# AhmedKishki/AMP-SPARC-SpatialModulation

Measured on AMD Instinct MI355X. Metric: detected symbol-vectors/sec, VAMP Nt=256 Nr=512 16-QAM; SER match vs ref, higher is better.
Workload: dtype bf16x3; 1 GPU; cfg4: VAMP Nt=256 Nr=512 Na=8 16QAM batch=4096 iterations<=20 EbN0=8.0 dB, one channel per batch; global_batch=4096, parallelism=epoch-shard x1 (independent epochs, one all-reduce of the error counters)

## Files before the change

### amp-sparc-spatialmodulation_amd/csrc/amp_persist.h

```cpp
#pragma once

#include <cfloat>

#include "amp_common.h"

namespace amp {

constexpr int PRING = 4;

typedef float f32x4 __attribute__((ext_vector_type(4)));
typedef unsigned u32x4 __attribute__((ext_vector_type(4)));

__device__ __forceinline__ f32x4 mfma16x16x4(float a, float b, f32x4 c) {
    return __builtin_amdgcn_mfma_f32_16x16x4f32(a, b, c, 0, 0, 0);
}

template <int NT, int G>
__device__ __forceinline__ void gemm16(const float* sA, int lda, const float* __restrict__ wq, int ct0,
                                       f32x4 (&acc)[NT]) {
    constexpr int R = G < PRING ? G : PRING;
    const int lane = threadIdx.x & 63;
#pragma unroll
    for (int t = 0; t < NT; ++t) acc[t] = f32x4{0.f, 0.f, 0.f, 0.f};
    const int ct0u = __builtin_amdgcn_readfirstlane(ct0);
    const __amdgpu_buffer_rsrc_t wr = __builtin_amdgcn_make_buffer_rsrc(
        const_cast<float*>(wq) + (size_t)ct0u * G * 256, (short)0, 0x7ffffff0, 0x00020000);
    const int vo = lane * 16;
    auto wload = [&](int t, int g) {
        const f32x4 v = __builtin_amdgcn_raw_buffer_load_b128(wr, vo, (t * G + g) * 1024, 0);
        return make_float4(v.x, v.y, v.z, v.w);
    };
    float4 ring[R][NT];
#pragma unroll
    for (int d = 0; d < R; ++d)
#pragma unroll
        for (int t = 0; t < NT; ++t) ring[d][t] = wload(t, d);
    const float* a_s = sA + (lane & 15) * lda + 4 * (lane >> 4);
    float4 acur = *reinterpret_cast<const float4*>(a_s);
#pragma unroll
    for (int g = 0; g < G; ++g) {
        const int d = g % R;
        const float4 anext = *reinterpret_cast<const float4*>(a_s + 16 * (g + 1 < G ? g + 1 : g));
#pragma unroll
        for (int t = 0; t < NT; ++t) acc[t] = mfma16x16x4(acur.x, ring[d][t].x, acc[t]);
#pragma unroll
        for (int t = 0; t < NT; ++t) acc[t] = mfma16x16x4(acur.y, ring[d][t].y, acc[t]);
#pragma unroll
        for (int t = 0; t < NT; ++t) acc[t] = mfma16x16x4(acur.z, ring[d][t].z, acc[t]);
#pragma unroll
        for (int t = 0; t < NT; ++t) acc[t] = mfma16x16x4(acur.w, ring[d][t].w, acc[t]);
        if (g + R < G) {
#pragma unroll
            for (int t = 0; t < NT; ++t) ring[d][t] = wload(t, g + R);
        }
        acur = anext;
        __builtin_amdgcn_sched_barrier(0);
    }
}

__host__ __device__ inline int pl_ldx(int K) { return K; }
__device__ __forceinline__ int pl_mask(int ldx) {
    const int n = ldx >> 3;
    const int b = n & -n;
    return (b < 16 ? b : 16) - 1;
}
__device__ __forceinline__ int pl_col(int row, int j, int m) { return j ^ ((row & m) << 3); }
__device__ __forceinline__ int pl_opaque(int x) {
#ifndef AMP_PL_HOIST
    asm volatile("" : "+v"(x));
#endif
    return x;
}

typedef const __attribute__((address_space(4))) char* KargPtr;
template <class A, class B>
constexpr int karg_second_offset() {
    return (int)((sizeof(A) + alignof(B) - 1) / alignof(B) * alignof(B));
}
template <class T>
__device__ __forceinline__ const T* karg_at(unsigned long long base, int off) {
    return (const T*)(const __attribute__((address_space(4))) T*)(KargPtr)(base + (unsigned long long)off);
}
__device__ __forceinline__ unsigned long long karg_launder(unsigned long long v) {
    asm volatile("" : "+s"(v));
    return v;
}
__device__ __forceinline__ unsigned long long karg_base() {
    return (unsigned long long)(KargPtr)__builtin_amdgcn_kernarg_segment_ptr();
}

typedef __bf16 bf16x8 __attribute__((ext_vector_type(8)));

typedef __bf16 bf16x2_t __attribute__((ext_vector_type(2)));
typedef float f32x2_t __attribute__((ext_vector_type(2)));

__device__ __forceinline__ void split3x2(float x, float y, unsigned& p0, unsigned& p1, unsigned& p2) {
    const f32x2_t v = {x, y};
    const bf16x2_t b0 = __builtin_convertvector(v, bf16x2_t);
    f32x2_t r1 = v - __builtin_convertvector(b0, f32x2_t);
    r1.x = __builtin_isfinite(x) ? r1.x : 0.0f;
    r1.y = __builtin_isfinite(y) ? r1.y : 0.0f;
    const bf16x2_t b1 = __builtin_convertvector(r1, bf16x2_t);
    const f32x2_t r2 = r1 - __builtin_convertvector(b1, f32x2_t);
    const bf16x2_t b2 = __builtin_convertvector(r2, bf16x2_t);
    p0 = __builtin_bit_cast(unsigned, b0);
    p1 = __builtin_bit_cast(unsigned, b1);
    p2 = __builtin_bit_cast(unsigned, b2);
}

__device__ __forceinline__ void x3_store8(unsigned short* sP, int ldx, int row, int j0, const float (&re)[8],
                                          const float (&im)[8]) {
    u32x4 q[6];
#pragma unroll
    for (int h = 0; h < 4; ++h) {
        unsigned a0, a1, a2, b0, b1, b2;
        split3x2(re[2 * h], re[2 * h + 1], a0, a1, a2);
        split3x2(im[2 * h], im[2 * h + 1], b0, b1, b2);
        q[0][h] = a0; q[1][h] = a1; q[2][h] = a2; q[3][h] = b0; q[4][h] = b1; q[5][h] = b2;
    }
    const int c = pl_col(pl_opaque(row), j0, pl_mask(ldx));
#pragma unroll
    for (int f = 0; f < 6; ++f) *reinterpret_cast<u32x4*>(sP + (f * 16 + row) * ldx + c) = q[f];
}

__device__ __forceinline__ float dpp_swap_pair(float v) {
    return __int_as_float(__builtin_amdgcn_update_dpp(0, __float_as_int(v), 0xB1, 0xF, 0xF, false));
}

__device__ __forceinline__ void x3_store_acc(unsigned short* sP, int ldx, int o, const float (&vr)[4],
                                             const float (&vi)[4]) {
    const int lane = pl_opaque((int)threadIdx.x) & 63;
    const bool odd = (lane & 1) != 0;
    float gr[2], gi[2];
#pragma unroll
    for (int h = 0; h < 2; ++h) {
        gr[h] = dpp_swap_pair(odd ? vr[h] : vr[2 + h]);
        gi[h] = dpp_swap_pair(odd ? vi[h] : vi[2 + h]);
    }
    const int row0 = 4 * (lane >> 4) + (odd ? 2 : 0);
    const int m = pl_mask(ldx);
    const int pl = 16 * ldx;
#pragma unroll
    for (int h = 0; h < 2; ++h) {
        unsigned short* p = sP + (row0 + h) * ldx + pl_col(row0 + h, o & ~1, m);
        const float mr = odd ? vr[2 + h] : vr[h], mi = odd ? vi[2 + h] : vi[h];
        unsigned q[6];
        split3x2(odd ? gr[h] : mr, odd ? mr : gr[h], q[0], q[1], q[2]);
        split3x2(odd ? gi[h] : mi, odd ? mi : gi[h], q[3], q[4], q[5]);
#pragma unroll
        for (int f = 0; f < 6; ++f) *reinterpret_cast<unsigned*>(p + f * pl) = q[f];
    }
}

__device__ __forceinline__ void split3(float x, unsigned& p0, unsigned& p1, unsigned& p2) {
    unsigned q0, q1, q2;
    split3x2(x, 0.0f, q0, q1, q2);
    p0 = q0 & 0xffffu; p1 = q1 & 0xffffu; p2 = q2 & 0xffffu;
}

__device__ __forceinline__ bf16x8 as_bf16x8(u32x4 v) { return __builtin_bit_cast(bf16x8, v); }

template <int NT, int G, int R = 1, bool PIN = false, bool HL = false>
__device__ __forceinline__ void gemm_x3(const unsigned short* sP, int ldx, const void* __restrict__ wq, int ct0,
                                        f32x4 (&cr)[NT], f32x4 (&ci)[NT]) {
    constexpr int RR = G < R ? G : R;
    constexpr int NL = HL ? NT : 1;
    const int lane = threadIdx.x & 63;
    f32x4 lr[NL], li[NL];
#pragma unroll
    for (int t = 0; t < NT; ++t) { cr[t] = f32x4{0.f, 0.f, 0.f, 0.f}; ci[t] = f32x4{0.f, 0.f, 0.f, 0.f}; }
#pragma unroll
    for (int t = 0; t < NL; ++t) { lr[t] = f32x4{0.f, 0.f, 0.f, 0.f}; li[t] = f32x4{0.f, 0.f, 0.f, 0.f}; }
    const int ct0u = __builtin_amdgcn_readfirstlane(ct0);
    const __amdgpu_buffer_rsrc_t wr = __builtin_amdgcn_make_buffer_rsrc(
        (char*)const_cast<void*>(wq) + (size_t)ct0u * G * 6 * 1024, (short)0, 0x7ffffff0, 0x00020000);
    const int vo = lane * 16;
    u32x4 ring[RR][NT][6];
#pragma unroll
    for (int d = 0; d < RR; ++d)
#pragma unroll
        for (int t = 0; t < NT; ++t)
#pragma unroll
            for (int f = 0; f < 6; ++f)
                ring[d][t][f] = __builtin_amdgcn_raw_buffer_load_b128(wr, vo, ((t * G + d) * 6 + f) * 1024, 0);
    const int ln = pl_opaque(lane);
    const int sw = (ln & 15) & pl_mask(ldx);
    const unsigned short* ap = sP + (ln & 15) * ldx + 8 * ((ln >> 4) ^ (sw & 3));
    const int s32 = 32 * (sw >> 2);
    const u32x4 sgn = {0x80008000u, 0x80008000u, 0x80008000u, 0x80008000u};
    u32x4 an[6];
    if constexpr (!PIN) {
#pragma unroll
        for (int f = 0; f < 6; ++f) an[f] = *reinterpret_cast<const u32x4*>(ap + s32 + f * 16 * ldx);
    }
#pragma unroll
    for (int g = 0; g < G; ++g) {
        const int d = g % RR;
        u32x4 a[6], na[3];
        if constexpr (PIN) {
#pragma unroll
            for (int f = 0; f < 6; ++f) a[f] = *reinterpret_cast<const u32x4*>(ap + ((32 * g) ^ s32) + f * 16 * ldx);
        } else {
#pragma unroll
            for (int f = 0; f < 6; ++f) a[f] = an[f];
            if (g + 1 < G) {
#pragma unroll
                for (int f = 0; f < 6; ++f)
                    an[f] = *reinterpret_cast<const u32x4*>(ap + ((32 * (g + 1)) ^ s32) + f * 16 * ldx);
            }
        }
#pragma unroll
        for (int f = 0; f < 3; ++f) na[f] = a[3 + f] ^ sgn;
#pragma unroll
        for (int t = 0; t < NT; ++t) {
            const u32x4* w = ring[d][t];
            f32x4 gr = cr[t], gi = ci[t];
            f32x4 sr = HL ? lr[HL ? t : 0] : gr, si = HL ? li[HL ? t : 0] : gi;
#define AMP_MF(acc, x, y) acc = __builtin_amdgcn_mfma_f32_16x16x32_bf16(as_bf16x8(x), as_bf16x8(y), acc, 0, 0, 0)
            AMP_MF(sr, a[0], w[2]);  AMP_MF(si, a[0], w[5]);
            AMP_MF(sr, a[1], w[1]);  AMP_MF(si, a[1], w[4]);
            AMP_MF(sr, a[2], w[0]);  AMP_MF(si, a[2], w[3]);
            AMP_MF(sr, na[0], w[5]); AMP_MF(si, a[3], w[2]);
            AMP_MF(sr, na[1], w[4]); AMP_MF(si, a[4], w[1]);
            AMP_MF(sr, na[2], w[3]); AMP_MF(si, a[5], w[0]);
            AMP_MF(sr, a[0], w[1]);  AMP_MF(si, a[0], w[4]);
            AMP_MF(sr, a[1], w[0]);  AMP_MF(si, a[1], w[3]);
            AMP_MF(sr, na[0], w[4]); AMP_MF(si, a[3], w[1]);
            AMP_MF(sr, na[1], w[3]); AMP_MF(si, a[4], w[0]);
            if constexpr (HL) {
                lr[HL ? t : 0] = sr; li[HL ? t : 0] = si;
            } else {
                gr = sr; gi = si;
            }
            AMP_MF(gr, a[0], w[0]);  AMP_MF(gi, a[0], w[3]);
            AMP_MF(gr, na[0], w[3]); AMP_MF(gi, a[3], w[0]);
#undef AMP_MF
            cr[t] = gr; ci[t] = gi;
        }
        if constexpr (PIN) __builtin_amdgcn_sched_barrier(0);
        if (g + RR < G) {
#pragma unroll
            for (int t = 0; t < NT; ++t)
#pragma unroll
                for (int f = 0; f < 6; ++f)
                    ring[d][t][f] = __builtin_amdgcn_raw_buffer_load_b128(wr, vo, ((t * G + g + RR) * 6 + f) * 1024, 0);
        }
        __builtin_amdgcn_sched_barrier(0);
    }
    if constexpr (HL) {
#pragma unroll
        for (int t = 0; t < NT; ++t) { cr[t] += lr[HL ? t : 0]; ci[t] += li[HL ? t : 0]; }
    }
}

typedef _Float16 f16x8 __attribute__((ext_vector_type(8)));
typedef _Float16 f16x2_t __attribute__((ext_vector_type(2)));
constexpr int H2_EX = 14;
constexpr int YH2_EX = 10;

__device__ __forceinline__ int h2_row_exp(float m) {
    if (!(m > 0.f) || !__builtin_isfinite(m)) return 0;
    return 14 - __builtin_amdgcn_frexp_expf(m);
}

__device__ __forceinline__ void split2x2(float x, float y, unsigned& p0, unsigned& p1) {
    const f32x2_t v = {x, y};
    const f16x2_t h0 = __builtin_convertvector(v, f16x2_t);
    const f32x2_t b = __builtin_convertvector(h0, f32x2_t);
    f32x2_t r = v - b;
    r.x = __builtin_isfinite(b.x) ? r.x : 0.0f;
    r.y = __builtin_isfinite(b.y) ? r.y : 0.0f;
    const f16x2_t h1 = __builtin_convertvector(r, f16x2_t);
    p0 = __builtin_bit_cast(unsigned, h0);
    p1 = __builtin_bit_cast(unsigned, h1);
}

__device__ __forceinline__ void split2(float x, int e, unsigned& p0, unsigned& p1) {
    unsigned q0, q1;
    split2x2(__builtin_amdgcn_ldexpf(x, e), 0.0f, q0, q1);
    p0 = q0 & 0xffffu; p1 = q1 & 0xffffu;
}

__device__ __forceinline__ void h2_store8(unsigned short* sP, int ldx, int row, int j0, const float (&re)[8],
                                          const float (&im)[8]) {
    u32x4 q[4];
#pragma unroll
    for (int h = 0; h < 4; ++h) {
        unsigned a0, a1, b0, b1;
        split2x2(re[2 * h], re[2 * h + 1], a0, a1);
        split2x2(im[2 * h], im[2 * h + 1], b0, b1);
        q[0][h] = a0; q[1][h] = a1; q[2][h] = b0; q[3][h] = b1;
    }
    const int c = pl_col(pl_opaque(row), j0, pl_mask(ldx));
#pragma unroll
    for (int f = 0; f < 4; ++f) *reinterpret_cast<u32x4*>(sP + (f * 16 + row) * ldx + c) = q[f];
}

__device__ __forceinline__ void h2_store_acc(unsigned short* sP, int ldx, int o, const float (&vr)[4],
                                             const float (&vi)[4]) {
    const int lane = pl_opaque((int)threadIdx.x) & 63;
    const bool odd = (lane & 1) != 0;
    float gr[2], gi[2];
#pragma unroll
    for (int h = 0; h < 2; ++h) {
        gr[h] = dpp_swap_pair(odd ? vr[h] : vr[2 + h]);
        gi[h] = dpp_swap_pair(odd ? vi[h] : vi[2 + h]);
    }
    const int row0 = 4 * (lane >> 4) + (odd ? 2 : 0);
    const int m = pl_mask(ldx);
    const int pl = 16 * ldx;
#pragma unroll
    for (int h = 0; h < 2; ++h) {
        unsigned short* p = sP + (row0 + h) * ldx + pl_col(row0 + h, o & ~1, m);
        const float mr = odd ? vr[2 + h] : vr[h], mi = odd ? vi[2 + h] : vi[h];
        unsigned q[4];
        split2x2(odd ? gr[h] : mr, odd ? mr : gr[h], q[0], q[1]);
        split2x2(odd ? gi[h] : mi, odd ? mi : gi[h], q[2], q[3]);
#pragma unroll
        for (int f = 0; f < 4; ++f) *reinterpret_cast<unsigned*>(p + f * pl) = q[f];
    }
}

__device__ __forceinline__ f16x8 as_f16x8(u32x4 v) { return __builtin_bit_cast(f16x8, v); }

template <int NT, int G, int R = 1>
__device__ __forceinline__ void gemm_h2(const unsigned short* sP, int ldx, const void* __restrict__ wq, int ct0,
                                        f32x4 (&cr)[NT], f32x4 (&ci)[NT]) {
    constexpr int RR = G < R ? G : R;
    const int lane = threadIdx.x & 63;
#pragma unroll
    for (int t = 0; t < NT; ++t) { cr[t] = f32x4{0.f, 0.f, 0.f, 0.f}; ci[t] = f32x4{0.f, 0.f, 0.f, 0.f}; }
    const int ct0u = __builtin_amdgcn_readfirstlane(ct0);
    const __amdgpu_buffer_rsrc_t wr = __builtin_amdgcn_make_buffer_rsrc(
        (char*)const_cast<void*>(wq) + (size_t)ct0u * G * 4 * 1024, (short)0, 0x7ffffff0, 0x00020000);
    const int vo = lane * 16;
    u32x4 ring[RR][NT][4];
#pragma unroll
    for (int d = 0; d < RR; ++d)
#pragma unroll
        for (int t = 0; t < NT; ++t)
#pragma unroll
            for (int f = 0; f < 4; ++f)
                ring[d][t][f] = __builtin_amdgcn_raw_buffer_load_b128(wr, vo, ((t * G + d) * 4 + f) * 1024, 0);
    const int ln = pl_opaque(lane);
    const int sw = (ln & 15) & pl_mask(ldx);
    const unsigned short* ap = sP + (ln & 15) * ldx + 8 * ((ln >> 4) ^ (sw & 3));
    const int s32 = 32 * (sw >> 2);
    const u32x4 sgn = {0x80008000u, 0x80008000u, 0x80008000u, 0x80008000u};
    u32x4 an[4];
#pragma unroll
    for (int f = 0; f < 4; ++f) an[f] = *reinterpret_cast<const u32x4*>(ap + s32 + f * 16 * ldx);
#pragma unroll
    for (int g = 0; g < G; ++g) {
        const int d = g % RR;
        u32x4 a[4], na[2];
#pragma unroll
        for (int f = 0; f < 4; ++f) a[f] = an[f];
        if (g + 1 < G) {
#pragma unroll
            for (int f = 0; f < 4; ++f)
                an[f] = *reinterpret_cast<const u32x4*>(ap + ((32 * (g + 1)) ^ s32) + f * 16 * ldx);
        }
#pragma unroll
        for (int f = 0; f < 2; ++f) na[f] = a[2 + f] ^ sgn;
#pragma unroll
        for (int t = 0; t < NT; ++t) {
            const u32x4* w = ring[d][t];
#define AMP_MH(acc, x, y) acc = __builtin_amdgcn_mfma_f32_16x16x32_f16(as_f16x8(x), as_f16x8(y), acc, 0, 0, 0)
            AMP_MH(cr[t], a[0], w[1]);  AMP_MH(ci[t], a[0], w[3]);
            AMP_MH(cr[t], a[1], w[0]);  AMP_MH(ci[t], a[1], w[2]);
            AMP_MH(cr[t], na[0], w[3]); AMP_MH(ci[t], a[2], w[1]);
            AMP_MH(cr[t], na[1], w[2]); AMP_MH(ci[t], a[3], w[0]);
            AMP_MH(cr[t], a[0], w[0]);  AMP_MH(ci[t], a[0], w[2]);
            AMP_MH(cr[t], na[0], w[2]); AMP_MH(ci[t], a[2], w[0]);
#undef AMP_MH
        }
        if (g + RR < G) {
#pragma unroll
            for (int t = 0; t < NT; ++t)
#pragma unroll
                for (int f = 0; f < 4; ++f)
                    ring[d][t][f] = __builtin_amdgcn_raw_buffer_load_b128(wr, vo, ((t * G + g + RR) * 4 + f) * 1024, 0);
        }
        __builtin_amdgcn_sched_barrier(0);
    }
}

typedef int i32x4 __attribute__((ext_vector_type(4)));
#ifndef AMP_I8_APF
#define AMP_I8_APF 1
#endif
__host__ __device__ __forceinline__ size_t i8_exp_offset(int O, int J) { return (size_t)O * J * 8; }

__host__ __device__ __forceinline__ int i8_ldb(int N) { return N + 16; }
__host__ __device__ __forceinline__ int i8_plane_floats(int N) { return 8 * 16 * i8_ldb(N) / 4; }

__device__ __forceinline__ int i8_row_exp(float m) {
    if (!(m <= FLT_MAX)) return 0x7fffffff;
    if (!(m > 0.f)) return 0;
    return __builtin_amdgcn_frexp_expf(m);
}
__device__ __forceinline__ float i8_absmax(float m, float v) {
    const float a = fabsf(v);
    return fmaxf(m, a <= FLT_MAX ? a : INFINITY);
}
// ... 262 lines not shown
```

### amp-sparc-spatialmodulation_amd/csrc/amp_vamp_persist_kernel.h

```cpp
#pragma once

#include <stdlib.h>

#include <type_traits>

#include "amp_decide_fused.h"
#include "amp_persist.h"
#include "amp_vamp.h"

namespace amp {

constexpr int AMP_TRACE_STRIDE = 10;
#ifndef AMP_OCC2_PK
#define AMP_OCC2_PK 0
#endif
#ifndef AMP_KK4_DU
#define AMP_KK4_DU 4
#endif
#ifndef AMP_X3_W8_PIN
#define AMP_X3_W8_PIN 0
#endif
#ifndef AMP_X3_W8_RING
#define AMP_X3_W8_RING 1
#endif
#ifndef AMP_X3_W8_PKGRID
#define AMP_X3_W8_PKGRID 1
#endif
#ifndef AMP_X3_DU
#define AMP_X3_DU 2
#endif

struct PLayout {
    int lda, ldr;
    int offA, offR, offX, offV0, offV1, offSM, offSA, offScr, total;
};

__host__ __device__ inline int x3_ldx(int N) { return pl_ldx(N); }
__host__ __device__ inline int x3_plane_floats(int N) { return 6 * 16 * x3_ldx(N) / 2; }

__host__ __device__ inline PLayout playout(int N, int k, int L, bool x3 = false) {
    PLayout y;
    y.lda = (2 * N > 2 * k ? 2 * N : 2 * k) + 4;
    y.ldr = 2 * N + (x3 ? 8 : 4);
    int o = 0;
    y.offA = o; o += (x3 && x3_plane_floats(N) > PBM * y.lda) ? x3_plane_floats(N) : PBM * y.lda;
    y.offR = o; o += PBM * y.ldr;
    y.offX = o; o += PBM * y.ldr;
    y.offV0 = o; o += PBM * N;
    y.offV1 = o; o += PBM * N;
    y.offSM = o; o += PBM * L;
    y.offSA = o; o += PBM * L;
    o = (o + 3) & ~3;
    y.offScr = o; o += 1024;
    y.total = o;
    return y;
}

constexpr int KARG_DC_OFF = karg_second_offset<VampK, DecConst>();

template <int NT, int KK, int NWV, int DU, bool X3, int OCC = 1, bool H2 = false, bool I8 = false>
__global__ __launch_bounds__(64 * NWV, OCC * NWV / 4) void vamp_persist(VampK P_arg, DecConst dc_arg) {
    (void)P_arg;
    (void)dc_arg;
    unsigned long long kbase = karg_base();
    const VampK* Pp = karg_at<VampK>(kbase, 0);
    const DecConst* Dp = karg_at<DecConst>(kbase, KARG_DC_OFF);
#define P (*Pp)
#define dc (*Dp)
    static_assert(!X3 || ((NWV == 4 || (NWV == 8 && !H2 && OCC == 1)) && NT % 2 == 0),
                  "X3: four waves (eight for the bf16x3 two-waves-per-SIMD form), whole complex tiles");
    static_assert(!(H2 && I8) && (!I8 || X3), "I8: a split-precision form of its own");
    constexpr int PKDEN = ((OCC * NWV / 4 == 1) || AMP_OCC2_PK) ? PK_ALL
                          : (NWV == 8 && KK == 16 && AMP_X3_W8_PKGRID) ? PK_GRID : PK_NONE;
    constexpr int PWG = 64 * NWV;
    constexpr int NC = X3 ? NT / 2 : 1;
    constexpr int G3 = NT * NWV / 4;
    constexpr int X3R = (NWV == 8) ? AMP_X3_W8_RING : 1;
    constexpr bool X3PIN = NWV == 8 && AMP_X3_W8_PIN;
#define c64 (static_cast<const Const64&>(*Dp))
    extern __shared__ __attribute__((aligned(16))) float lds[];
    __shared__ int s_flag;
    __shared__ double s_d[PWG / 64][4];
    __shared__ float s_hmax[PWG / 64][PBM];
    __shared__ int s_hexp[PBM];
    const PLayout Y = playout(P.N, P.k, P.L, X3);
    float* sA = lds + Y.offA;
    float* sR = lds + Y.offR;
    float* sX = lds + Y.offX;
    float* sM = lds + Y.offSM;
    float* sS = lds + Y.offSA;
    float* scr = lds + Y.offScr;
    const int tid = threadIdx.x, lane = tid & 63, wave = tid >> 6;
    const int wg = blockIdx.x, nwg = gridDim.x;
    const int wgx = wg + P.wg_off, nwx = P.nwg_x;
    const int ep = wgx / P.wpe, wl = wgx - ep * P.wpe, wg0 = ep * P.wpe;
    const int lrow0 = wl * PBM;
    const int row0 = ep * P.B + lrow0 - P.row_off, nrows = min(PBM, P.B - lrow0);
#define ebar (P.pbar + (P.E > 1 ? PBAR_EPOCH + ep : 0))
    const int N = P.N, twoN = 2 * N, twok = 2 * P.k, M = P.M, spr = N / M;
    const float* const sv_ep = P.s + (size_t)ep * P.sch;
#define Wx1 ((const void*)((const char*)P.Wx1 + ep * P.wch))
#define Wx2 ((const void*)((const char*)P.Wx2 + ep * P.wch))
    const int ldr = Y.ldr, lda = Y.lda;
    const int ct0 = wave * NT;
    const int cc0 = wave * NC;
    unsigned short* sP = reinterpret_cast<unsigned short*>(sA);
    const int ldx = x3_ldx(N);
    signed char* sB = reinterpret_cast<signed char*>(sA);
    const int ldb = i8_ldb(N);

    float yt[NT][4], s2c[NT];
#pragma unroll
    for (int t = 0; t < NT; ++t) {
        const int col = X3 ? 2 * (16 * (cc0 + (t < NC ? t : 0)) + (lane & 15)) : 16 * (ct0 + t) + (lane & 15);
        const float sv = sv_ep[col >> 1];
        s2c[t] = sv * sv;
    }
    if (H2 && P.ytil_in_kernel) {
      if constexpr (H2) {
        constexpr int IPY = NT / 2;
        const int n = P.n, ldy = pl_ldx(n);
        const int row = tid % PBM;
        float re[IPY][8], im[IPY][8];
        float m = 0.f;
#pragma unroll
        for (int i = 0; i < IPY; ++i) {
            const int e = tid + i * PWG;
            const int j0 = 8 * (e / PBM);
#pragma unroll
            for (int h = 0; h < 4; ++h) {
                float4 v = *reinterpret_cast<const float4*>(P.y + (size_t)(row0 + max(min(row, nrows - 1), 0)) * 2 * n + 2 * j0 + 4 * h);
                if (!(row < nrows)) v = make_float4(0.f, 0.f, 0.f, 0.f);
                re[i][2 * h] = v.x; im[i][2 * h] = v.y; re[i][2 * h + 1] = v.z; im[i][2 * h + 1] = v.w;
            }
#pragma unroll
            for (int h = 0; h < 8; ++h) m = fmaxf(m, fmaxf(fabsf(re[i][h]), fabsf(im[i][h])));
        }
        m = fmaxf(m, __shfl_xor(m, 16));
        m = fmaxf(m, __shfl_xor(m, 32));
        if (lane < PBM) s_hmax[wave][lane] = m;
        __syncthreads();
        float mr = s_hmax[0][row];
#pragma unroll
        for (int w = 1; w < PWG / 64; ++w) mr = fmaxf(mr, s_hmax[w][row]);
        const int ex = h2_row_exp(mr);
        if (tid < PBM) s_hexp[tid] = ex;
#pragma unroll
        for (int i = 0; i < IPY; ++i) {
            const int e = tid + i * PWG;
#pragma unroll
            for (int h = 0; h < 8; ++h) {
                re[i][h] = __builtin_amdgcn_ldexpf(re[i][h], ex);
                im[i][h] = __builtin_amdgcn_ldexpf(im[i][h], ex);
            }
            h2_store8(sP, ldy, row, 8 * (e / PBM), re[i], im[i]);
        }
        __syncthreads();
        f32x4 yr[NC], yi[NC];
        gemm_h2<NC, 2 * G3>(sP, ldy, P.Wq0, cc0, yr, yi);
#pragma unroll
        for (int r = 0; r < 4; ++r) {
            const float sc = __builtin_amdgcn_ldexpf(1.0f, -(s_hexp[4 * (lane >> 4) + r] + YH2_EX));
#pragma unroll
            for (int t = 0; t < NC; ++t) {
                yt[2 * t][r] = yr[t][r] * sc;
                yt[2 * t + 1][r] = yi[t][r] * sc;
            }
        }
        __syncthreads();
      }
    } else if (X3) {
      if constexpr (!I8) {
#pragma unroll
        for (int t = 0; t < NC; ++t) {
            const int o = 16 * (cc0 + t) + (lane & 15);
#pragma unroll
            for (int r = 0; r < 4; ++r) {
                const int row = 4 * (lane >> 4) + r;
                const bool in = row < nrows;
                const size_t yo = (size_t)(row0 + max(min(row, nrows - 1), 0)) * twok + 2 * o;
                const float a = P.ytil[yo], b = P.ytil[yo + 1];
                yt[2 * t][r] = in ? a : 0.f;
                yt[2 * t + 1][r] = in ? b : 0.f;
            }
        }
      }
    } else if (P.ytil_in_kernel) {
        const int ldy = 4 * N + 4;
        for (int e = tid; e < PBM * N; e += PWG) {
            const int row = e / N, c4 = 4 * (e - row * N);
            float4 v = *reinterpret_cast<const float4*>(P.y + (size_t)(row0 + max(min(row, nrows - 1), 0)) * 4 * N + c4);
            if (!(row < nrows)) v = make_float4(0.f, 0.f, 0.f, 0.f);
            *reinterpret_cast<float4*>(lds + row * ldy + c4) = v;
        }
        __syncthreads();
        f32x4 acc[NT];
        gemm16<NT, 2 * NT * NWV>(lds, ldy, P.Wq0, ct0, acc);
#pragma unroll
        for (int t = 0; t < NT; ++t)
#pragma unroll
            for (int r = 0; r < 4; ++r) yt[t][r] = acc[t][r];
        __syncthreads();
    } else {
#pragma unroll
        for (int t = 0; t < NT; ++t) {
            const int col = 16 * (ct0 + t) + (lane & 15);
#pragma unroll
            for (int r = 0; r < 4; ++r) {
                const int row = 4 * (lane >> 4) + r;
                const float yv = P.ytil[(size_t)(row0 + max(min(row, nrows - 1), 0)) * twok + col];
                yt[t][r] = (row < nrows) ? yv : 0.f;
            }
        }
    }
    VampIter cur;
    {
        const S2Lane s2l = s2_lane(P, sv_ep);
        cur = vamp_first_iter(P, scr, &s2l);
    }
    {
        const float p = (float)P.sparsity;
        for (int e = tid; e < PBM * twoN; e += PWG) {
            const int row = e / twoN, col = e - row * twoN;
            sR[row * ldr + col] = 0.f;
            sX[row * ldr + col] = (row < nrows && (col & 1) == 0) ? p : 0.f;
        }
        for (int e = tid; e < PBM * N; e += PWG) lds[Y.offV1 + e] = 1.0f;
    }

    unsigned long long* trc = P.trace;
    auto stamp = [&](int t, int ph) {
        if (trc && tid == 0 && t < P.max_iter) trc[((size_t)wg * P.max_iter + t) * AMP_TRACE_STRIDE + ph] = __builtin_amdgcn_s_memtime();
    };
    if (trc && tid == 0) {
        trc[(size_t)nwg * P.max_iter * AMP_TRACE_STRIDE + 2 * wg] = __builtin_amdgcn_s_memtime();
        trc[(size_t)nwg * P.max_iter * AMP_TRACE_STRIDE + 2 * wg + 1] = __builtin_amdgcn_s_memrealtime();
    }
    unsigned nbar = 0;
#define grs (gran_rsrc(P.pparts, (unsigned)(P.max_iter * nwx) * 32u))
    int fixed = 0, last_t = 0, aborted = 0;
    VampIter nx = cur;
    auto exchange = [&](int te, float* vnew, const float* vprev) -> bool {
            PartAcc g;
            const S2Lane s2x = s2_lane(P, P.s + (size_t)ep * P.sch);
            const unsigned tag = P.gen * (unsigned)(P.max_iter + 1) + (unsigned)te + 1u;
            if (!part_gather(grs, ((unsigned)te * nwx + wg0) * 32u, P.wpe, tag, P.pbar + 1, g, scr, &s_flag)) return false;
            stamp(te, 6);
            fixed = 0;
            if (part_allnan(g)) {
                if (!cur.fixed_all) {
                    const float qn = __int_as_float(0x7fc00000);
                    for (int e = tid; e < nrows * twoN; e += PWG) sX[(e / twoN) * ldr + e % twoN] = qn;
                    for (int e = tid; e < nrows * N; e += PWG) vnew[e] = qn;
                }
                g.sumvar = __longlong_as_double(0x7ff8000000000000LL);
                g.notclose = 1;
                fixed = -1;
            } else if (part_danger(g)) {
                const double G32 = g.maxabs, slack = logit_slack(G32);
                const float inv = cur.inv_sigma2;
                auto ldf = [=](int s) {
                    const int row = s / spr, sj = s - row * spr;
                    const float* rp = sR + row * ldr + 2 * sj * M;
                    return [=](int m, float& rr, float& ri, float& it) {
                        rr = rp[2 * m]; ri = rp[2 * m + 1]; it = inv;
                    };
                };
                double gm = 0.0;
                for (int s = tid; s < nrows * spr; s += PWG)
                    if ((double)sS[s] >= G32 - slack) gm = fmax(gm, section_absmax_f64(ldf(s), M, c64));
                gm = group_max(gm, 64);
                if (lane == 0) s_d[wave][0] = gm;
                __syncthreads();
                if (tid == 0) {
                    double m4 = 0.0;
                    for (int w = 0; w < PWG / 64; ++w) m4 = fmax(m4, s_d[w][0]);
                    P.pxch[((size_t)te * nwx + wgx) * 4 + 0] = m4;
                }
                if (!grid_sync_on(ebar, P.pbar + 1, ++nbar * (unsigned)P.wpe, &s_flag)) return false;
                double G = 0.0;
                for (int w = wg0; w < wg0 + P.wpe; ++w) G = fmax(G, P.pxch[((size_t)te * nwx + w) * 4 + 0]);
                double dsum = 0.0;
                int dnc = 0, cnt = 0;
                for (int s = tid; s < nrows * spr; s += PWG) {
                    if (!((double)sM[s] - G < AMP_DANGER + slack)) continue;
                    ++cnt;
                    const int row = s / spr, sj = s - row * spr;
                    float* xp = sX + row * ldr + 2 * sj * M;
                    const int v0 = row * N + sj * M;
                    auto st = [&](int m, float xr, float xi, float var) {
                        const float old = vnew[v0 + m];
                        dsum += (double)var - (double)old;
                        dnc += (torch_close(var, vprev[v0 + m]) ? 0 : 1) - (torch_close(old, vprev[v0 + m]) ? 0 : 1);
                        xp[2 * m] = xr; xp[2 * m + 1] = xi;
                        vnew[v0 + m] = var;
                    };
                    exact_section_f64<true>(ldf(s), st, M, c64, G);
                }
                dsum = group_sum(dsum, 64);
                dnc = group_sum(dnc, 64);
                cnt = group_sum(cnt, 64);
                __syncthreads();
                if (lane == 0) { s_d[wave][1] = dsum; s_d[wave][2] = (double)dnc; s_d[wave][3] = (double)cnt; }
                __syncthreads();
                if (tid == 0) {
                    double a = 0.0, b = 0.0, c = 0.0;
                    for (int w = 0; w < PWG / 64; ++w) { a += s_d[w][1]; b += s_d[w][2]; c += s_d[w][3]; }
                    P.pxch[((size_t)te * nwx + wgx) * 4 + 1] = a;
                    P.pxch[((size_t)te * nwx + wgx) * 4 + 2] = b;
                    P.pxch[((size_t)te * nwx + wgx) * 4 + 3] = c;
                }
                if (!grid_sync_on(ebar, P.pbar + 1, ++nbar * (unsigned)P.wpe, &s_flag)) return false;
                double a = 0.0, b = 0.0, c = 0.0;
                for (int w = wg0; w < wg0 + P.wpe; ++w) {
                    const double* q = P.pxch + ((size_t)te * nwx + w) * 4;
                    a += q[1]; b += q[2]; c += q[3];
                }
                g.sumvar += a;
                g.notclose = (uint32_t)((long long)g.notclose + (long long)b);
                g.maxabs = G;
                fixed = (int)c;
            }
        stamp(te, 9);
        nx = vamp_advance(P, cur, g, fixed, te, scr, &s2x);
        stamp(te, 7);
        return true;
    };

    for (int t = 0; t < P.max_iter; ++t) {
        kbase = karg_launder(kbase);
        Pp = karg_at<VampK>(kbase, 0);
        Dp = karg_at<DecConst>(kbase, KARG_DC_OFF);
        last_t = t;
        stamp(t, 0);
        const float* vprev = lds + ((t & 1) ? Y.offV0 : Y.offV1);
        float* vnew = lds + ((t & 1) ? Y.offV1 : Y.offV0);
        f32x4 acc[NT];
        f32x4 cr[NC], ci[NC];
        if (__builtin_expect(X3 && !H2 && !I8 && t == 0 && P.q0_load != 0, 0)) {
            stamp(t, 1);
            const int lnq = pl_opaque(lane);
#pragma unroll
            for (int t2 = 0; t2 < NC; ++t2) {
                const float2 q = *reinterpret_cast<const float2*>(P.q0 + 2 * (16 * (cc0 + t2) + (lnq & 15)));
#pragma unroll
                for (int r = 0; r < 4; ++r) {
                    const bool in = 4 * (lnq >> 4) + r < nrows;
                    cr[t2][r] = in ? q.x : 0.f;
                    ci[t2][r] = in ? q.y : 0.f;
                }
            }
        } else {
        if constexpr (H2 || I8) {
            constexpr int IPT = (NT + 3) / 4;
            const int tdp = I8 ? pl_opaque(tid) : tid;
            const int row = tdp % PBM;
            float re[IPT][8], im[IPT][8];
            float m = 0.f;
#pragma unroll
            for (int i = 0; i < IPT; ++i) {
                const int e = tdp + i * PWG;
                const int j0 = 8 * (e / PBM);
                const bool ok = e < PBM * (N >> 3);
#pragma unroll
                for (int h = 0; h < 4; ++h) {
                    float4 x = make_float4(0.f, 0.f, 0.f, 0.f), q = x;
                    if (ok) {
                        x = *reinterpret_cast<const float4*>(sX + row * ldr + 2 * j0 + 4 * h);
                        q = *reinterpret_cast<const float4*>(sR + row * ldr + 2 * j0 + 4 * h);
                    }
                    re[i][2 * h] = (x.x - cur.dxdr_prev * q.x) * cur.ns_prev;
                    im[i][2 * h] = (x.y - cur.dxdr_prev * q.y) * cur.ns_prev;
                    re[i][2 * h + 1] = (x.z - cur.dxdr_prev * q.z) * cur.ns_prev;
                    im[i][2 * h + 1] = (x.w - cur.dxdr_prev * q.w) * cur.ns_prev;
                }
#pragma unroll
                for (int h = 0; h < 8; ++h) {
                    if constexpr (I8) m = i8_absmax(i8_absmax(m, re[i][h]), im[i][h]);
                    else m = fmaxf(m, fmaxf(fabsf(re[i][h]), fabsf(im[i][h])));
                }
            }
            m = fmaxf(m, __shfl_xor(m, 16));
            m = fmaxf(m, __shfl_xor(m, 32));
            if (lane < PBM) s_hmax[wave][lane] = m;
            __syncthreads();
            float mr = s_hmax[0][row];
#pragma unroll
            for (int w = 1; w < PWG / 64; ++w) mr = fmaxf(mr, s_hmax[w][row]);
            const int ex = I8 ? i8_row_exp(mr) : h2_row_exp(mr);
            if (tid < PBM) s_hexp[tid] = ex;
#pragma unroll
            for (int i = 0; i < IPT; ++i) {
                const int e = tdp + i * PWG;
                if (e < PBM * (N >> 3)) {
                    if constexpr (I8) {
                        i8_store8(sB, ldb, row, 8 * (e / PBM), re[i], im[i], ex);
                    } else {
#pragma unroll
                        for (int h = 0; h < 8; ++h) {
                            re[i][h] = __builtin_amdgcn_ldexpf(re[i][h], ex);
                            im[i][h] = __builtin_amdgcn_ldexpf(im[i][h], ex);
                        }
                        h2_store8(sP, ldx, row, 8 * (e / PBM), re[i], im[i]);
                    }
                }
            }
        } else if constexpr (X3) {
            const int tdx = NWV == 8 ? pl_opaque(tid) : tid;
            for (int e = tdx; e < PBM * (N >> 3); e += PWG) {
                const int row = e % PBM, j0 = 8 * (e / PBM);
                float re[8], im[8];
#pragma unroll
                for (int h = 0; h < 4; ++h) {
                    const float4 x = *reinterpret_cast<const float4*>(sX + row * ldr + 2 * j0 + 4 * h);
                    const float4 q = *reinterpret_cast<const float4*>(sR + row * ldr + 2 * j0 + 4 * h);
                    re[2 * h] = (x.x - cur.dxdr_prev * q.x) * cur.ns_prev;
                    im[2 * h] = (x.y - cur.dxdr_prev * q.y) * cur.ns_prev;
                    re[2 * h + 1] = (x.z - cur.dxdr_prev * q.z) * cur.ns_prev;
                    im[2 * h + 1] = (x.w - cur.dxdr_prev * q.w) * cur.ns_prev;
                }
                x3_store8(sP, ldx, row, j0, re, im);
            }
        } else
        for (int e = tid; e < PBM * (twoN >> 2); e += PWG) {
            const int row = e / (twoN >> 2), c4 = 4 * (e - row * (twoN >> 2));
            const float4 x = *reinterpret_cast<const float4*>(sX + row * ldr + c4);
            const float4 q = *reinterpret_cast<const float4*>(sR + row * ldr + c4);
            *reinterpret_cast<float4*>(sA + row * lda + c4) =
                make_float4((x.x - cur.dxdr_prev * q.x) * cur.ns_prev, (x.y - cur.dxdr_prev * q.y) * cur.ns_prev,
                            (x.z - cur.dxdr_prev * q.z) * cur.ns_prev, (x.w - cur.dxdr_prev * q.w) * cur.ns_prev);
        }
        __syncthreads();
        stamp(t, 1);
        if constexpr (I8) {
            float rowf[4];
#pragma unroll
            for (int r = 0; r < 4; ++r) rowf[r] = i8_row_factor(s_hexp[4 * (lane >> 4) + r]);
            gemm_i8<NC, G3 / 2>(sB, ldb, Wx1, N, cc0, rowf, cr, ci);
        } else if constexpr (H2)
            gemm_h2<NC, G3>(sP, ldx, Wx1, cc0, cr, ci);
        else if constexpr (X3) {
            gemm_x3<NC, G3, X3R, X3PIN, true>(sP, ldx, Wx1, cc0, cr, ci);
            if (__builtin_expect(t == 0 && P.q0_store != 0 && wg == 0, 0)) {
                const int lns = pl_opaque(lane);
                if (lns < 16) {
#pragma unroll
                    for (int t2 = 0; t2 < NC; ++t2)
                        *reinterpret_cast<float2*>(P.q0 + 2 * (16 * (cc0 + t2) + lns)) = make_float2(cr[t2][0], ci[t2][0]);
                }
            }
        } else
            gemm16<NT, NT * NWV>(sA, lda, P.Wq1, ct0, acc);
        }
        float hsc[4];
        int hew[4];
        if constexpr (H2 || I8) {
#pragma unroll
            for (int r = 0; r < 4; ++r) hsc[r] = I8 ? 1.0f : __builtin_amdgcn_ldexpf(1.0f, -(s_hexp[4 * (lane >> 4) + r] + H2_EX));
            float mrow[4] = {0.f, 0.f, 0.f, 0.f};
#pragma unroll
            for (int t2 = 0; t2 < NC; ++t2) {
                const float sc = 1.0f / (s2c[t2] + cur.vr);
                float ytr[4], yti[4];
                if constexpr (I8) {
                    const int ln = pl_opaque(lane);
                    const int oo = 16 * (cc0 + t2) + (ln & 15);
#pragma unroll
                    for (int r = 0; r < 4; ++r) {
                        const int row = 4 * (ln >> 4) + r;
                        const float2 u = *reinterpret_cast<const float2*>(P.ytil + (size_t)(row0 + max(min(row, nrows - 1), 0)) * twok + 2 * oo);
                        const float2 v = row < nrows ? u : make_float2(0.f, 0.f);
                        ytr[r] = v.x; yti[r] = v.y;
                    }
                } else {
#pragma unroll
                    for (int r = 0; r < 4; ++r) { ytr[r] = yt[2 * t2][r]; yti[r] = yt[2 * t2 + 1][r]; }
                }
#pragma unroll
                for (int r = 0; r < 4; ++r) {
                    const float qr = I8 ? cr[t2][r] : cr[t2][r] * hsc[r], qi = I8 ? ci[t2][r] : ci[t2][r] * hsc[r];
                    cr[t2][r] = sc * (ytr[r] + cur.vr * qr) - qr;
                    ci[t2][r] = sc * (yti[r] + cur.vr * qi) - qi;
                    if constexpr (I8) mrow[r] = i8_absmax(i8_absmax(mrow[r], cr[t2][r]), ci[t2][r]);
                    else mrow[r] = fmaxf(mrow[r], fmaxf(fabsf(cr[t2][r]), fabsf(ci[t2][r])));
                }
            }
#pragma unroll
            for (int r = 0; r < 4; ++r) {
#pragma unroll
                for (int sh = 1; sh < 16; sh <<= 1) mrow[r] = fmaxf(mrow[r], __shfl_xor(mrow[r], sh));
            }
            if ((lane & 15) == 0) {
#pragma unroll
                for (int r = 0; r < 4; ++r) s_hmax[wave][4 * (lane >> 4) + r] = mrow[r];
            }
        }
        __syncthreads();
        stamp(t, 2);
        if constexpr (H2 || I8) {
#pragma unroll
            for (int r = 0; r < 4; ++r) {
                float mr = s_hmax[0][4 * (lane >> 4) + r];
#pragma unroll
                for (int w = 1; w < PWG / 64; ++w) mr = fmaxf(mr, s_hmax[w][4 * (lane >> 4) + r]);
                hew[r] = I8 ? i8_row_exp(mr) : h2_row_exp(mr);
            }
            const int lnw = I8 ? pl_opaque(lane) : lane;
#pragma unroll
            for (int t2 = 0; t2 < NC; ++t2) {
                const int o = 16 * (cc0 + t2) + (lnw & 15);
                if constexpr (I8) {
                    int wr[4], wi[4];
#pragma unroll
                    for (int r = 0; r < 4; ++r) { wr[r] = i8_fix(cr[t2][r], hew[r]); wi[r] = i8_fix(ci[t2][r], hew[r]); }
                    i8_store_acc(sB, ldb, o, wr, wi);
                } else {
                    float wr[4], wi[4];
#pragma unroll
                    for (int r = 0; r < 4; ++r) {
                        wr[r] = __builtin_amdgcn_ldexpf(cr[t2][r], hew[r]);
                        wi[r] = __builtin_amdgcn_ldexpf(ci[t2][r], hew[r]);
                    }
                    h2_store_acc(sP, ldx, o, wr, wi);
                }
                if (P.dump) {
                    float* dp = P.dump + (((size_t)t * nwg + wg) * 5 + 0) * PBM * twoN;
#pragma unroll
                    for (int r = 0; r < 4; ++r) {
                        dp[(4 * (lane >> 4) + r) * twoN + 2 * o] = cr[t2][r];
                        dp[(4 * (lane >> 4) + r) * twoN + 2 * o + 1] = ci[t2][r];
                    }
                }
            }
#pragma unroll
            for (int r = 0; r < 4; ++r) hsc[r] = I8 ? i8_row_factor(hew[r]) : __builtin_amdgcn_ldexpf(1.0f, -(hew[r] + H2_EX));
        } else if constexpr (X3) {
            const int lnx = NWV == 8 ? pl_opaque(lane) : lane;
#pragma unroll
            for (int t2 = 0; t2 < NC; ++t2) {
                const int o = 16 * (cc0 + t2) + (lnx & 15);
                const float sc = 1.0f / (s2c[t2] + cur.vr);
                float wr[4], wi[4];
#pragma unroll
                for (int r = 0; r < 4; ++r) {
                    const float qr = cr[t2][r], qi = ci[t2][r];
                    wr[r] = sc * (yt[2 * t2][r] + cur.vr * qr) - qr;
                    wi[r] = sc * (yt[2 * t2 + 1][r] + cur.vr * qi) - qi;
                }
                x3_store_acc(sP, ldx, o, wr, wi);
                if (P.dump) {
                    float* dp = P.dump + (((size_t)t * nwg + wg) * 5 + 0) * PBM * twoN;
#pragma unroll
                    for (int r = 0; r < 4; ++r) {
                        dp[(4 * (lane >> 4) + r) * twoN + 2 * o] = wr[r];
                        dp[(4 * (lane >> 4) + r) * twoN + 2 * o + 1] = wi[r];
                    }
                }
            }
        } else
#pragma unroll
        for (int t2 = 0; t2 < NT; ++t2) {
            const int col = 16 * (ct0 + t2) + (lane & 15);
            const float sc = 1.0f / (s2c[t2] + cur.vr);
#pragma unroll
            for (int r = 0; r < 4; ++r) {
                const float q = acc[t2][r];
                sA[(4 * (lane >> 4) + r) * lda + col] = sc * (yt[t2][r] + cur.vr * q) - q;
            }
        }
        __syncthreads();
        stamp(t, 3);
        kbase = karg_launder(kbase);
        Pp = karg_at<VampK>(kbase, 0);
        Dp = karg_at<DecConst>(kbase, KARG_DC_OFF);
        auto r_epi = [&](int ccs, auto& er, auto& ei) __attribute__((always_inline)) {
            constexpr int NCX = std::extent<std::remove_reference_t<decltype(er)>>::value;
            const int lnr = (I8 || NWV == 8) ? pl_opaque(lane) : lane;
#pragma unroll
            for (int t2 = 0; t2 < NCX; ++t2) {
                const int o = 16 * (ccs + t2) + (lnr & 15);
#pragma unroll
                for (int r = 0; r < 4; ++r) {
                    const int b = (4 * (lnr >> 4) + r) * ldr + 2 * o;
                    const float rtr = (sX[b] - cur.dxdr_prev * sR[b]) * cur.ns_prev;
                    const float rti = (sX[b + 1] - cur.dxdr_prev * sR[b + 1]) * cur.ns_prev;
                    const float xtr = er[t2][r] + rtr, xti = ei[t2][r] + rti;
                    sR[b] = (xtr - cur.alpha * rtr) * cur.inv1ma;
                    sR[b + 1] = (xti - cur.alpha * rti) * cur.inv1ma;
                    if (P.dump) {
                        float* dp = P.dump + (((size_t)t * nwg + wg) * 5 + 1) * PBM * twoN;
                        dp[(4 * (lane >> 4) + r) * twoN + 2 * o] = sR[b];
                        dp[(4 * (lane >> 4) + r) * twoN + 2 * o + 1] = sR[b + 1];
                    }
                }
            }
        };
        if constexpr (X3) {
            if constexpr (I8) {
                gemm_i8<NC, G3 / 2>(sB, ldb, Wx2, N, cc0, hsc, cr, ci);
            } else if constexpr (H2) {
                gemm_h2<NC, G3>(sP, ldx, Wx2, cc0, cr, ci);
#pragma unroll
                for (int t2 = 0; t2 < NC; ++t2)
#pragma unroll
                    for (int r = 0; r < 4; ++r) { cr[t2][r] *= hsc[r]; ci[t2][r] *= hsc[r]; }
            }
            if constexpr (!I8 && !H2) gemm_x3<NC, G3, X3R, X3PIN, true>(sP, ldx, Wx2, cc0, cr, ci);
            r_epi(cc0, cr, ci);
        } else {
        gemm16<NT, NT * NWV>(sA, lda, P.Wq2, ct0, acc);
#pragma unroll
        for (int t2 = 0; t2 < NT; ++t2) {
            const int col = 16 * (ct0 + t2) + (lane & 15);
#pragma unroll
            for (int r = 0; r < 4; ++r) {
                const int o = (4 * (lane >> 4) + r) * ldr + col;
                const float rt = (sX[o] - cur.dxdr_prev * sR[o]) * cur.ns_prev;
                const float xt = acc[t2][r] + rt;
                sR[o] = (xt - cur.alpha * rt) * cur.inv1ma;
            }
        }
        }
        __syncthreads();
        PDenoisePolicy pol{sR, sX, vnew, vprev, sM, sS, ldr, M, 31 - __builtin_clz(spr), N, cur.inv_sigma2};
        if (P.dump) pol.dbg = P.dump + (((size_t)t * nwg + wg) * 5 + 4) * PBM * twoN;
        PartAcc pa;
        kbase = karg_launder(kbase);
        Pp = karg_at<VampK>(kbase, 0);
        Dp = karg_at<DecConst>(kbase, KARG_DC_OFF);
        stamp(t, 4);
        if constexpr (KK > 16)
            denoise_sections_wide_m<true, KK>(pol, nrows * spr, M, P.c, pa);
        else
            denoise_sections_u<true, KK, DU, PKDEN>(pol, nrows * spr, M, P.c, pa);
        stamp(t, 8);
        const unsigned tag = P.gen * (unsigned)(P.max_iter + 1) + (unsigned)t + 1u;
        part_publish(pa, grs, ((unsigned)t * nwx + wgx) * 32u, tag, scr);
        if (P.dump) {
            float* dp = P.dump + (((size_t)t * nwg + wg) * 5 + 2) * PBM * twoN;
            for (int e = tid; e < PBM * twoN; e += PWG) dp[e] = sX[(e / twoN) * ldr + e % twoN];
            for (int e = tid; e < PBM * N; e += PWG) dp[PBM * twoN + (e / N) * twoN + e % N] = vnew[e];
            if (tid == 0) {
                const Partial* sp = reinterpret_cast<const Partial*>(scr);
                for (int w = 0; w < PWG / 64; ++w) {
                    double v = sp[w].sumvar;
                    __builtin_memcpy(dp + PBM * twoN + N + 2 * w, &v, 8);
                }
                dp[PBM * twoN + twoN + N] = cur.inv_sigma2;
            }
        }
        stamp(t, 5);
        kbase = karg_launder(kbase);
        Pp = karg_at<VampK>(kbase, 0);
        Dp = karg_at<DecConst>(kbase, KARG_DC_OFF);
        if (!exchange(t, vnew, vprev)) { aborted = 1; break; }
        if (nx.stopped || t + 1 == P.max_iter) break;
        cur = nx;
    }
    __syncthreads();
    if (trc && tid == 0) {
        trc[(size_t)nwg * P.max_iter * AMP_TRACE_STRIDE + 2 * nwg + 2 * wg] = __builtin_amdgcn_s_memtime();
        trc[(size_t)nwg * P.max_iter * AMP_TRACE_STRIDE + 2 * nwg + 2 * wg + 1] = __builtin_amdgcn_s_memrealtime();
    }
    const float* vlast = lds + ((last_t & 1) ? Y.offV1 : Y.offV0);
    for (int e = tid; e < nrows * twoN; e += PWG) {
        const int row = e / twoN, col = e - row * twoN;
        P.r[(size_t)(row0 + row) * twoN + col] = sR[row * ldr + col];
        P.xm[(size_t)(row0 + row) * twoN + col] = sX[row * ldr + col];
    }
    for (int e = tid; e < nrows * N; e += PWG) P.var0[(size_t)row0 * N + e] = vlast[e];
    amp_status st_rec = vamp_make_status(P, cur, nx, fixed);
    if (aborted) st_rec.nan_state = -1;
    if (wl == P.wg_off && tid == 0) P.status[ep] = st_rec;
    if (P.dec_on) {
        __syncthreads();
        const unsigned dtag = P.fold_in ? P.gen * (unsigned)(P.max_iter + 1) + (unsigned)P.max_iter + 1u : 0u;
        decide_epilogue<PWG, KK, true>(P, dc, sR, sX, ldr, row0, lrow0, nrows, sA, lds + Y.offV0,
                                       4 * (Y.offScr - Y.offV0), scr, dtag);
        const int nloc = nwg / P.E;
        if (P.fold_in && wg % nloc == 0) {
            __syncthreads();
            const bool ok = dec_fold_gather(P, wg, nloc, dtag, P.counts + ep, scr, &s_flag);
            if (tid == 0) {
                if (!ok) {
                    st_rec.nan_state = -1;
                    P.status[ep] = st_rec;
                }
                if (P.host_rec && P.E == 1) host_record_write(P.host_rec, st_rec, P.counts[ep]);
            }
        }
    }
#undef P
#undef dc
#undef c64
#undef ebar
#undef Wx1
#undef Wx2
#undef grs
}

int device_cu_count();

template <int NT, int KK, int NWV, int DU, bool X3, int OCC = 1, bool H2 = false, bool I8 = false>
static int persist_launch_t(const VampK& P, const DecConst& dc, hipStream_t st) {
    const void* fn = (const void*)vamp_persist<NT, KK, NWV, DU, X3, OCC, H2, I8>;
    const size_t lds = (size_t)playout(P.N, P.k, P.L, X3).total * 4;
    static size_t attr_lds = 0;
    static int per_cu = 0;
    hipError_t e = hipSuccess;
    if (attr_lds != lds) {
        e = hipFuncSetAttribute(fn, hipFuncAttributeMaxDynamicSharedMemorySize, (int)lds);
        if (e != hipSuccess) {
            set_error("vamp_persist: hipFuncSetAttribute: %s", hipGetErrorString(e));
            return AMP_E_LAUNCH;
        }
        e = hipOccupancyMaxActiveBlocksPerMultiprocessor(&per_cu, fn, 64 * NWV, lds);
        if (e != hipSuccess) per_cu = 0;
        attr_lds = lds;
    }
    VampK Pc = P;
    DecConst dd = dc;
    void* args[] = {(void*)&Pc, (void*)&dd};
    return persist_grid_launch("vamp_persist", fn, P.nwg, 64 * NWV, lds, per_cu, args, st);
}

template <int NT, int NWV, bool X3, int OCC = 1, bool H2 = false, bool I8 = false>
static int persist_launch_nt(const VampK& P, const DecConst& dc, hipStream_t st) {
    switch (P.c.K) {
    case 1: return persist_launch_t<NT, 1, NWV, 4, X3, OCC, H2, I8>(P, dc, st);
    case 2: return persist_launch_t<NT, 2, NWV, 4, X3, OCC, H2, I8>(P, dc, st);
    case 4: return persist_launch_t<NT, 4, NWV, AMP_KK4_DU, X3, OCC, H2, I8>(P, dc, st);
    case 8: return persist_launch_t<NT, 8, NWV, 2, X3, OCC, H2, I8>(P, dc, st);
    case 16:
        return persist_launch_t<NT, 16, NWV, X3 ? AMP_X3_DU : 2, X3, OCC, H2, I8>(P, dc, st);
    default: return persist_launch_t<NT, 64, NWV, 1, X3, OCC, H2, I8>(P, dc, st);
    }
}

}
```

Measured before the change: 6.089 million symbol-vectors/s.

## Prefetch X3 weight ring across operator boundaries and overlap with LDS staging

Refactors the bf16x3 GEMM so its weight register ring can be filled outside the call. The first operator's ring is filled in two halves around the LDS staging of the activation planes. The tail of the first GEMM then prefetches the second operator's leading weight groups into the freed slots. This is meant to hide global weight-load latency at GEMM start and between the two GEMMs, at the cost of more live registers across the staging loop and the code between the GEMMs.

Result: faster. 6.200 million symbol-vectors/s (median of 6 runs) (+1.8%).

```diff
diff --git a/amp-sparc-spatialmodulation_amd/csrc/amp_persist.h b/amp-sparc-spatialmodulation_amd/csrc/amp_persist.h
--- a/amp-sparc-spatialmodulation_amd/csrc/amp_persist.h
+++ b/amp-sparc-spatialmodulation_amd/csrc/amp_persist.h
@@ -160,10 +160,45 @@
 
 __device__ __forceinline__ bf16x8 as_bf16x8(u32x4 v) { return __builtin_bit_cast(bf16x8, v); }
 
-template <int NT, int G, int R = 1, bool PIN = false, bool HL = false>
-__device__ __forceinline__ void gemm_x3(const unsigned short* sP, int ldx, const void* __restrict__ wq, int ct0,
-                                        f32x4 (&cr)[NT], f32x4 (&ci)[NT]) {
-    constexpr int RR = G < R ? G : R;
+constexpr int x3_ring_depth(int G, int R) { return G < R ? G : R; }
+template <int NT, int RR>
+struct X3Ring {
+    u32x4 v[RR][NT][6];
+};
+
+template <int G>
+__device__ __forceinline__ __amdgpu_buffer_rsrc_t x3_wrsrc(const void* wq, int ct0) {
+    const int ct0u = __builtin_amdgcn_readfirstlane(ct0);
+    return __builtin_amdgcn_make_buffer_rsrc((char*)const_cast<void*>(wq) + (size_t)ct0u * G * 6 * 1024, (short)0,
+                                             0x7ffffff0, 0x00020000);
+}
+
+template <int NT, int G, int RR, int T0 = 0, int T1 = NT>
+__device__ __forceinline__ void x3_ring_load(X3Ring<NT, RR>& ring, int d, __amdgpu_buffer_rsrc_t wr, int g) {
+    const int vo = (threadIdx.x & 63) * 16;
+#pragma unroll
+    for (int t = T0; t < T1; ++t)
+#pragma unroll
+        for (int f = 0; f < 6; ++f)
+            ring.v[d][t][f] = __builtin_amdgcn_raw_buffer_load_b128(wr, vo, ((t * G + g) * 6 + f) * 1024, 0);
+}
+
+template <int NT, int G, int R = 1, int T0 = 0, int T1 = NT>
+__device__ __forceinline__ void x3_ring_fill(X3Ring<NT, x3_ring_depth(G, R)>& ring, const void* __restrict__ wq, int ct0) {
+    const __amdgpu_buffer_rsrc_t wr = x3_wrsrc<G>(wq, ct0);
+#pragma unroll
+    for (int d = 0; d < x3_ring_depth(G, R); ++d) x3_ring_load<NT, G, x3_ring_depth(G, R), T0, T1>(ring, d, wr, d);
+}
+
+struct X3NoHook {
+    __device__ __forceinline__ void operator()(int) const {}
+};
+template <int NT, int G, int R = 1, bool PIN = false, bool HL = false, bool NEXT = false, class Hook = X3NoHook>
+__device__ __forceinline__ void gemm_x3_ring(const unsigned short* sP, int ldx, const void* __restrict__ wq, int ct0,
+                                             X3Ring<NT, x3_ring_depth(G, R)>& ring, f32x4 (&cr)[NT], f32x4 (&ci)[NT],
+                                             const void* __restrict__ wq_next = nullptr, Hook&& hook = Hook()) {
+    constexpr int RR = x3_ring_depth(G, R);
+    static_assert(!NEXT || G % RR == 0, "the next operator's group j lands in slot j % RR");
     constexpr int NL = HL ? NT : 1;
     const int lane = threadIdx.x & 63;
     f32x4 lr[NL], li[NL];
@@ -171,18 +206,7 @@
     for (int t = 0; t < NT; ++t) { cr[t] = f32x4{0.f, 0.f, 0.f, 0.f}; ci[t] = f32x4{0.f, 0.f, 0.f, 0.f}; }
 #pragma unroll
     for (int t = 0; t < NL; ++t) { lr[t] = f32x4{0.f, 0.f, 0.f, 0.f}; li[t] = f32x4{0.f, 0.f, 0.f, 0.f}; }
-    const int ct0u = __builtin_amdgcn_readfirstlane(ct0);
-    const __amdgpu_buffer_rsrc_t wr = __builtin_amdgcn_make_buffer_rsrc(
-        (char*)const_cast<void*>(wq) + (size_t)ct0u * G * 6 * 1024, (short)0, 0x7ffffff0, 0x00020000);
-    const int vo = lane * 16;
-    u32x4 ring[RR][NT][6];
-#pragma unroll
-    for (int d = 0; d < RR; ++d)
-#pragma unroll
-        for (int t = 0; t < NT; ++t)
-#pragma unroll
-            for (int f = 0; f < 6; ++f)
-                ring[d][t][f] = __builtin_amdgcn_raw_buffer_load_b128(wr, vo, ((t * G + d) * 6 + f) * 1024, 0);
+    const __amdgpu_buffer_rsrc_t wr = x3_wrsrc<G>(wq, ct0);
     const int ln = pl_opaque(lane);
     const int sw = (ln & 15) & pl_mask(ldx);
     const unsigned short* ap = sP + (ln & 15) * ldx + 8 * ((ln >> 4) ^ (sw & 3));
@@ -213,7 +237,7 @@
         for (int f = 0; f < 3; ++f) na[f] = a[3 + f] ^ sgn;
 #pragma unroll
         for (int t = 0; t < NT; ++t) {
-            const u32x4* w = ring[d][t];
+            const u32x4* w = ring.v[d][t];
             f32x4 gr = cr[t], gi = ci[t];
             f32x4 sr = HL ? lr[HL ? t : 0] : gr, si = HL ? li[HL ? t : 0] : gi;
 #define AMP_MF(acc, x, y) acc = __builtin_amdgcn_mfma_f32_16x16x32_bf16(as_bf16x8(x), as_bf16x8(y), acc, 0, 0, 0)
@@ -238,12 +262,11 @@
             cr[t] = gr; ci[t] = gi;
         }
         if constexpr (PIN) __builtin_amdgcn_sched_barrier(0);
+        hook(g);
         if (g + RR < G) {
-#pragma unroll
-            for (int t = 0; t < NT; ++t)
-#pragma unroll
-                for (int f = 0; f < 6; ++f)
-                    ring[d][t][f] = __builtin_amdgcn_raw_buffer_load_b128(wr, vo, ((t * G + g + RR) * 6 + f) * 1024, 0);
+            x3_ring_load<NT, G>(ring, d, wr, g + RR);
+        } else if constexpr (NEXT) {
+            x3_ring_load<NT, G>(ring, d, x3_wrsrc<G>(wq_next, ct0), g + RR - G);
         }
         __builtin_amdgcn_sched_barrier(0);
     }
@@ -251,6 +274,14 @@
 #pragma unroll
         for (int t = 0; t < NT; ++t) { cr[t] += lr[HL ? t : 0]; ci[t] += li[HL ? t : 0]; }
     }
+}
+
+template <int NT, int G, int R = 1, bool PIN = false, bool HL = false>
+__device__ __forceinline__ void gemm_x3(const unsigned short* sP, int ldx, const void* __restrict__ wq, int ct0,
+                                        f32x4 (&cr)[NT], f32x4 (&ci)[NT]) {
+    X3Ring<NT, x3_ring_depth(G, R)> ring;
+    x3_ring_fill<NT, G, R>(ring, wq, ct0);
+    gemm_x3_ring<NT, G, R, PIN, HL>(sP, ldx, wq, ct0, ring, cr, ci);
 }
 
 typedef _Float16 f16x8 __attribute__((ext_vector_type(8)));
diff --git a/amp-sparc-spatialmodulation_amd/csrc/amp_vamp_persist_kernel.h b/amp-sparc-spatialmodulation_amd/csrc/amp_vamp_persist_kernel.h
--- a/amp-sparc-spatialmodulation_amd/csrc/amp_vamp_persist_kernel.h
+++ b/amp-sparc-spatialmodulation_amd/csrc/amp_vamp_persist_kernel.h
@@ -77,6 +77,8 @@
     constexpr int G3 = NT * NWV / 4;
     constexpr int X3R = (NWV == 8) ? AMP_X3_W8_RING : 1;
     constexpr bool X3PIN = NWV == 8 && AMP_X3_W8_PIN;
+    constexpr bool X3PF = X3 && !H2 && !I8;
+    constexpr int PFT = (NC + 1) / 2;
 #define c64 (static_cast<const Const64&>(*Dp))
     extern __shared__ __attribute__((aligned(16))) float lds[];
     __shared__ int s_flag;
@@ -337,6 +339,7 @@
         float* vnew = lds + ((t & 1) ? Y.offV1 : Y.offV0);
         f32x4 acc[NT];
         f32x4 cr[NC], ci[NC];
+        X3Ring<NC, x3_ring_depth(G3, X3R)> wring;
         if (__builtin_expect(X3 && !H2 && !I8 && t == 0 && P.q0_load != 0, 0)) {
             stamp(t, 1);
             const int lnq = pl_opaque(lane);
@@ -350,6 +353,7 @@
                     ci[t2][r] = in ? q.y : 0.f;
                 }
             }
+            x3_ring_fill<NC, G3, X3R>(wring, Wx2, cc0);
         } else {
         if constexpr (H2 || I8) {
             constexpr int IPT = (NT + 3) / 4;
@@ -406,6 +410,10 @@
                 }
             }
         } else if constexpr (X3) {
+            if constexpr (X3PF) {
+                x3_ring_fill<NC, G3, X3R, 0, PFT>(wring, Wx1, cc0);
+                __builtin_amdgcn_sched_barrier(0);
+            }
             const int tdx = NWV == 8 ? pl_opaque(tid) : tid;
             for (int e = tdx; e < PBM * (N >> 3); e += PWG) {
                 const int row = e % PBM, j0 = 8 * (e / PBM);
@@ -420,6 +428,10 @@
                     im[2 * h + 1] = (x.w - cur.dxdr_prev * q.w) * cur.ns_prev;
                 }
                 x3_store8(sP, ldx, row, j0, re, im);
+            }
+            if constexpr (X3PF) {
+                __builtin_amdgcn_sched_barrier(0);
+                x3_ring_fill<NC, G3, X3R, PFT, NC>(wring, Wx1, cc0);
             }
         } else
         for (int e = tid; e < PBM * (twoN >> 2); e += PWG) {
@@ -440,7 +452,7 @@
         } else if constexpr (H2)
             gemm_h2<NC, G3>(sP, ldx, Wx1, cc0, cr, ci);
         else if constexpr (X3) {
-            gemm_x3<NC, G3, X3R, X3PIN, true>(sP, ldx, Wx1, cc0, cr, ci);
+            gemm_x3_ring<NC, G3, X3R, X3PIN, true, true>(sP, ldx, Wx1, cc0, wring, cr, ci, Wx2);
             if (__builtin_expect(t == 0 && P.q0_store != 0 && wg == 0, 0)) {
                 const int lns = pl_opaque(lane);
                 if (lns < 16) {
@@ -605,7 +617,7 @@
 #pragma unroll
                     for (int r = 0; r < 4; ++r) { cr[t2][r] *= hsc[r]; ci[t2][r] *= hsc[r]; }
             }
-            if constexpr (!I8 && !H2) gemm_x3<NC, G3, X3R, X3PIN, true>(sP, ldx, Wx2, cc0, cr, ci);
+            if constexpr (X3PF) gemm_x3_ring<NC, G3, X3R, X3PIN, true>(sP, ldx, Wx2, cc0, wring, cr, ci);
             r_epi(cc0, cr, ci);
         } else {
         gemm16<NT, NT * NWV>(sA, lda, P.Wq2, ct0, acc);
```
